# HanielUlises/GCN-GrabCut

Measured on AMD Instinct MI355X. Metric: images/sec end-to-end mask (DUTS-shape batch), higher is better.
Workload: dtype f32

## Files before the change

### gcn-grabcut_amd/csrc/ggc_debug.hip

```cpp
#include "ggc_internal.h"

extern "C" int ggc_debug_read_scratch(ggc_ctx* ctx, const char* name, void* host_dst, size_t bytes) {
    if (!ctx || !name || !host_dst) return GGC_E_INVALID_ARG;
    static const struct { const char* n; int slot; } tab[] = {
        {"slic_raw_labels", ggc::S_SLIC_LABELS}, {"slic_centers", ggc::S_SLIC_CENTERS},
        {"slic_image_a", ggc::S_SLIC_IMG}, {"slic_image_b", ggc::S_SLIC_TMP}, {"slic_stale", ggc::S_SLIC_AUX2},
        {"grabcut_comp", ggc::S_GC_D}, {"grabcut_nweights", ggc::S_GC_E}, {"grabcut_gmm", ggc::S_GC_B},
        {"grabcut_excess_sink_dist", ggc::S_GC_G},
        {"net_states", ggc::S_STATES}, {"net_xw", ggc::S_XW}, {"net_agg", ggc::S_AGG}, {"net_hjk", ggc::S_HJK},
        {"net_score", ggc::S_SCORE}, {"net_gvec", ggc::S_GVEC}, {"net_gate", ggc::S_GATE},
        {"scissors_planes", ggc::S_SCISSORS},
    };
    for (auto& t : tab)
        if (std::strcmp(t.n, name) == 0) {
            const ggc::Buf& b = ctx->slots[t.slot];
            GGC_REQUIRE(ctx, b.p && b.bytes >= bytes, GGC_E_STATE, "scratch '%s' holds %zu bytes, asked for %zu", name,
                        b.bytes, bytes);
            GGC_HIP(ctx, hipSetDevice(ctx->device));
            GGC_HIP(ctx, hipDeviceSynchronize());
            GGC_HIP(ctx, hipMemcpy(host_dst, b.p, bytes, hipMemcpyDeviceToHost));
            return GGC_OK;
        }
    return ggc::set_err(ctx, GGC_E_INVALID_ARG, "unknown scratch name '%s'", name);
}
```

### gcn-grabcut_amd/csrc/ggc_gc.h

```cpp
#pragma once
#include "ggc_internal.h"

namespace ggc {

constexpr int DINF = 1 << 29;

struct GcDims { int B, H, W, P, n_chunks; };

__device__ __forceinline__ int dir_dx(int dir) { return (dir == 0 || dir == 4 || dir == 7) ? -1 : ((dir == 1 || dir == 5 || dir == 6) ? 1 : 0); }
__device__ __forceinline__ int dir_dy(int dir) { return (dir == 2 || dir == 4 || dir == 6) ? -1 : ((dir == 3 || dir == 5 || dir == 7) ? 1 : 0); }
__device__ __forceinline__ int dir_nb(const GcDims& d, int y, int x, int dir) {
    const int yy = y + dir_dy(dir), xx = x + dir_dx(dir);
    if (xx < 0 || xx >= d.W || yy < 0 || yy >= d.H) return -1;
    return yy * d.W + xx;
}

__host__ __device__ __forceinline__ size_t rc_idx(int dir, size_t i) { return i * 8 + (size_t)dir; }

__device__ __forceinline__ void mf_init_pixel(const GcDims& d, int b, int p, int32_t tw, const int32_t* __restrict__ nw,
                                              int32_t* __restrict__ rc, int32_t* __restrict__ ex, int32_t* __restrict__ snk,
                                              uint8_t* __restrict__ rmask, bool warm) {
    const size_t BP = (size_t)d.B * d.P, i = (size_t)b * d.P + p;
    const int y = p / d.W, x = p % d.W;
    const int32_t* nwb = nw + (size_t)b * d.P;
    const int dirs[4] = {0, 4, 2, 6};
    int32_t inflow = 0;
    int arcs = 0;
#pragma unroll
    for (int k = 0; k < 4; ++k) {
        const int dir = dirs[k];
        const int32_t c0 = dir_nb(d, y, x, dir) >= 0 ? nwb[(size_t)k * BP + p] : 0;
        const int q = dir_nb(d, y, x, dir ^ 1);
        const int32_t c1 = q >= 0 ? nwb[(size_t)k * BP + q] : 0;
        if (warm) {
            const int32_t ra = rc[rc_idx(dir, i)], rb = rc[rc_idx((dir ^ 1), i)];
            inflow += (ra - c0) + (rb - c1);
            arcs |= (ra > 0 ? 1 << dir : 0) | (rb > 0 ? 1 << (dir ^ 1) : 0);
        } else {
            rc[rc_idx(dir, i)] = c0;
            rc[rc_idx((dir ^ 1), i)] = c1;
            arcs |= (c0 > 0 ? 1 << dir : 0) | (c1 > 0 ? 1 << (dir ^ 1) : 0);
        }
    }
    rmask[i] = (uint8_t)arcs;
    const int32_t bal = tw + inflow;
    ex[i] = bal > 0 ? bal : 0;
    snk[i] = bal < 0 ? -bal : 0;
}

struct MfControl {
    int32_t* active;
    int32_t* cnt;
    int32_t* lists;
    int32_t* err;
};

int maxflow(ggc_ctx* ctx, hipStream_t st, const GcDims& d, const int32_t* state, int32_t* rc, int32_t* ex,
            int32_t* snk, int32_t* dist, uint8_t* rmask, const MfControl& ctl, bool masks_exact);

constexpr int MF_RT = 32;
constexpr int MF_PT_W = 32, MF_PT_H = 8;
struct MfTiles { int rt_x, rt_y, pt_x, pt_y; };

void mf_zero3(hipStream_t st, int32_t* a, size_t na, int32_t* b, size_t nb, int32_t* c, size_t nc);

constexpr int AQ_HEAD = 0, AQ_TAIL = 32, AQ_PENDING = 64, AQ_DONE = 96, AQ_BUDGET = 97, AQ_VISITS = 128, AQ_WORDS = 160;
int maxflow_relax_async(ggc_ctx* ctx, hipStream_t st, const GcDims& d, const MfTiles& tl, uint8_t* rmask, int32_t* dirty, const int32_t* rc, int32_t* dist,
                        const int32_t* count, const int32_t* list, int32_t* flag, unsigned long long* ring, int32_t* q, int cap,
                        int grid, int32_t* err_flag);
int maxflow_push_async(ggc_ctx* ctx, hipStream_t st, const GcDims& d, const MfTiles& tl, int th, int inner, int gen_max, int32_t* rc,
                       int32_t* ex, int32_t* snk, int32_t* dist, uint8_t* rmask, int32_t* dirty, const int32_t* count, const int32_t* list, int n_list_max, int32_t* state,
                       unsigned long long* ring, int32_t* q, int waves, int32_t* err_flag, long long* prof = nullptr);

}
```

### gcn-grabcut_amd/csrc/ggc_grabcut.hip

```cpp
#include "ggc_gc.h"
#include "ggc_math.h"
#include <algorithm>
#include <cmath>
#include <cstdlib>
#include <vector>

namespace ggc {

constexpr int NCOMP = 5;
constexpr double CAP_SCALE = 262144.0;
constexpr double GAMMA = 50.0, LAMBDA = 9.0 * GAMMA;
constexpr int CHUNK = 1024;


struct Gmm {
    double coef[NCOMP], mean[NCOMP][3], cov[NCOMP][9];
    double inv[NCOMP][3][3], det[NCOMP];
    double isd[NCOMP];
};

__host__ __device__ inline void gmm_prepare(Gmm& g, int ci, double fix) {
    if (!(g.coef[ci] > 0.0)) return;
    double* c = g.cov[ci];
    double d = c[0] * (c[4] * c[8] - c[5] * c[7]) - c[1] * (c[3] * c[8] - c[5] * c[6]) + c[2] * (c[3] * c[7] - c[4] * c[6]);
// ... 182 lines not shown
    }
    const uint64_t r = splitmix(rng);
    const bool by_d2 = k > 0 && total > 0;
    const long long t = by_d2 ? (long long)(r % (uint64_t)total) : (long long)(r % (uint64_t)n);
    const int64_t* w = by_d2 ? cd : cc;
    long long run = 0;
    int ch = d.n_chunks - 1;
    for (int base = 0; base < d.n_chunks; base += 64) {
        const int i = base + lane;
        const long long v = i < d.n_chunks ? (long long)w[i] : 0;
        const long long incl = wave_scan64(v, lane);
        const unsigned long long hit = __ballot(i < d.n_chunks && run + incl > t);
        if (hit) {
            const int l = __ffsll((long long)hit) - 1;
            ch = base + l;
            run += __shfl(incl - v, l, 64);
            break;
        }
        run += __shfl(incl, 63, 64);
    }
    if (ch == d.n_chunks - 1) {
        long long part = 0;
        for (int i = lane; i < d.n_chunks - 1; i += 64) part += w[i];
        run = wave_sum64(part);
    }
    int pick = -1, last = -1;
    const int p_end = min((ch + 1) * CHUNK, d.P);
    for (int base = ch * CHUNK; base < p_end; base += 64) {
        const int p = base + lane;
        const bool mine = p < p_end && (is_bg(mask[(size_t)b * d.P + p]) ? 0 : 1) == c;
        const long long v = mine ? (by_d2 ? (long long)d2[(size_t)b * d.P + p] : 1) : 0;
        const long long incl = wave_scan64(v, lane);
        const unsigned long long any = __ballot(mine);
        if (any) last = base + 63 - __clzll((long long)any);
        const unsigned long long hit = __ballot(mine && run + incl > t);
        if (hit) { pick = base + __ffsll((long long)hit) - 1; break; }
        run += __shfl(incl, 63, 64);
    }
    if (pick < 0) pick = last;
    if (lane == 0) {
        s.rng = rng;
        s.cen_px[k] = pick;
        for (int ch3 = 0; ch3 < 3; ++ch3) s.cen[k][ch3] = (double)img[((size_t)b * d.P + pick) * 3 + ch3];
    }
}

constexpr int ACC_W = 13;

constexpr int BIN_COPIES = 16, BIN_PX = 4;

__global__ void __launch_bounds__(256) k_km_assign(GcDims d, const uint8_t* __restrict__ img,
                                                   const uint8_t* __restrict__ mask, const int32_t* __restrict__ state,
                                                   const KmState* __restrict__ km, uint8_t* __restrict__ comp,
                                                   unsigned long long* __restrict__ acc) {
    __shared__ unsigned int s_acc[2 * NCOMP * 4 * BIN_COPIES];
    const int b = blockIdx.y, tid = threadIdx.x, cp = tid % BIN_COPIES;
    if (state[b]) return;
    for (int i = tid; i < 2 * NCOMP * 4 * BIN_COPIES; i += 256) s_acc[i] = 0;
    __syncthreads();
#pragma unroll
    for (int j = 0; j < BIN_PX; ++j) {
        const int p = (blockIdx.x * BIN_PX + j) * 256 + tid;
        if (p < d.P) {
            const size_t gp = (size_t)b * d.P + p;
            const int c = is_bg(mask[gp]) ? 0 : 1;
            const uint8_t* px = img + gp * 3;
            int best = 0; double bd = 0.0;
#pragma unroll
            for (int cc = 0; cc < 2; ++cc) {
                if (c != cc) continue;
                const KmState& s = km[b * 2 + cc];
                for (int k = 0; k < s.K; ++k) {
                    const double a0 = (double)px[0] - s.cen[k][0], a1 = (double)px[1] - s.cen[k][1], a2 = (double)px[2] - s.cen[k][2];
                    const double dist = (a0 * a0 + a1 * a1) + a2 * a2;
                    if (k == 0 || dist < bd) { best = k; bd = dist; }
                }
            }
            comp[gp] = (uint8_t)best;
            unsigned int* a = s_acc + (c * NCOMP + best) * 4 * BIN_COPIES + cp;
            atomicAdd(&a[0], 1u); atomicAdd(&a[BIN_COPIES], (unsigned int)px[0]);
            atomicAdd(&a[2 * BIN_COPIES], (unsigned int)px[1]); atomicAdd(&a[3 * BIN_COPIES], (unsigned int)px[2]);
        }
    }
    __syncthreads();
    for (int i = tid; i < 2 * NCOMP * 4; i += 256) {
        unsigned int v = 0;
#pragma unroll
        for (int k = 0; k < BIN_COPIES; ++k) v += s_acc[i * BIN_COPIES + k];
        if (v) atomicAdd(&acc[((size_t)b * 2 * NCOMP + i / 4) * ACC_W + (i % 4)], (unsigned long long)v);
    }
}

__global__ void k_km_update(int B, const int32_t* __restrict__ state, KmState* __restrict__ km,
                            unsigned long long* __restrict__ acc, int update) {
    const int i = blockIdx.x * blockDim.x + threadIdx.x;
    if (i >= B * 2 * NCOMP) return;
    const int b = i / (2 * NCOMP), c = (i / NCOMP) % 2, k = i % NCOMP;
    unsigned long long* a = acc + (size_t)i * ACC_W;
    if (!state[b] && update && a[0] > 0)
        for (int ch = 0; ch < 3; ++ch) km[b * 2 + c].cen[k][ch] = (double)(long long)a[1 + ch] / (double)(long long)a[0];
    for (int j = 0; j < ACC_W; ++j) a[j] = 0;
}

template <int MODE>
__global__ void __launch_bounds__(256) k_gmm_accum(GcDims d, const uint8_t* __restrict__ img,
                                                   const uint8_t* __restrict__ mask, const int32_t* __restrict__ state,
                                                   const Gmm* __restrict__ gmm, uint8_t* __restrict__ comp,
                                                   unsigned long long* __restrict__ acc) {
    constexpr int LW = 10;
    __shared__ unsigned int s_acc[2 * NCOMP * LW * BIN_COPIES];
    const int b = blockIdx.y, tid = threadIdx.x, cp = tid % BIN_COPIES;
    if (state[b]) return;
    for (int i = tid; i < 2 * NCOMP * LW * BIN_COPIES; i += 256) s_acc[i] = 0;
    __syncthreads();
#pragma unroll
    for (int j = 0; j < BIN_PX; ++j) {
        const int p = (blockIdx.x * BIN_PX + j) * 256 + tid;
        if (p < d.P) {
            const size_t gp = (size_t)b * d.P + p;
            const int c = is_bg(mask[gp]) ? 0 : 1;
            const uint8_t* px = img + gp * 3;
            int ci = 0;
            if (MODE == 1) {
#pragma unroll
                for (int cc = 0; cc < 2; ++cc) if (c == cc) ci = gmm_which(gmm[b * 2 + cc], px);
                comp[gp] = (uint8_t)ci;
            } else ci = comp[gp];
            unsigned int* a = s_acc + (c * NCOMP + ci) * LW * BIN_COPIES + cp;
            const unsigned int v0 = px[0], v1 = px[1], v2 = px[2];
            atomicAdd(&a[0], 1u);
            atomicAdd(&a[1 * BIN_COPIES], v0); atomicAdd(&a[2 * BIN_COPIES], v1); atomicAdd(&a[3 * BIN_COPIES], v2);
            atomicAdd(&a[4 * BIN_COPIES], v0 * v0); atomicAdd(&a[5 * BIN_COPIES], v0 * v1); atomicAdd(&a[6 * BIN_COPIES], v0 * v2);
            atomicAdd(&a[7 * BIN_COPIES], v1 * v1); atomicAdd(&a[8 * BIN_COPIES], v1 * v2); atomicAdd(&a[9 * BIN_COPIES], v2 * v2);
        }
    }
    __syncthreads();
    for (int i = tid; i < 2 * NCOMP * ACC_W; i += 256) {
        const int bin = i / ACC_W, slot = i % ACC_W;
        int ls = slot;
        if (slot >= 4) {
            const int r = (slot - 4) / 3, cc = (slot - 4) % 3;
            const int lo = r < cc ? r : cc, hi = r < cc ? cc : r;
            ls = 4 + (lo == 0 ? hi : (lo == 1 ? 2 + hi : 5));
        }
        unsigned int v = 0;
#pragma unroll
        for (int k = 0; k < BIN_COPIES; ++k) v += s_acc[(bin * LW + ls) * BIN_COPIES + k];
        if (v) atomicAdd(&acc[(size_t)b * 2 * NCOMP * ACC_W + i], (unsigned long long)v);
    }
}

__global__ void k_gmm_learn(int B, const int32_t* __restrict__ state, unsigned long long* __restrict__ acc,
                            Gmm* __restrict__ gmm) {
    const int i = blockIdx.x * blockDim.x + threadIdx.x;
    if (i >= B * 2) return;
    unsigned long long* a = acc + (size_t)i * NCOMP * ACC_W;
    if (!state[i / 2]) {
        Gmm& g = gmm[i];
        long long total = 0;
        for (int ci = 0; ci < NCOMP; ++ci) total += (long long)a[ci * ACC_W];
        for (int ci = 0; ci < NCOMP; ++ci) {
            const long long n = (long long)a[ci * ACC_W];
            if (n == 0) { g.coef[ci] = 0.0; continue; }
            const double inv_n = 1.0 / (double)n;
            g.coef[ci] = (double)n / (double)total;
            for (int r = 0; r < 3; ++r) g.mean[ci][r] = (double)(long long)a[ci * ACC_W + 1 + r] * inv_n;
            for (int r = 0; r < 3; ++r)
                for (int c = 0; c < 3; ++c)
                    g.cov[ci][3 * r + c] = (double)(long long)a[ci * ACC_W + 4 + 3 * r + c] * inv_n - g.mean[ci][r] * g.mean[ci][c];
            gmm_prepare(g, ci, 0.01);
        }
    }
    for (int j = 0; j < NCOMP * ACC_W; ++j) a[j] = 0;
}

__global__ void k_gmm_from_model(int B, const double* __restrict__ bgd, const double* __restrict__ fgd, Gmm* __restrict__ gmm) {
    const int i = blockIdx.x * blockDim.x + threadIdx.x;
    if (i >= B * 2) return;
    const double* m = (i & 1 ? fgd : bgd) + (size_t)(i / 2) * 65;
    Gmm& g = gmm[i];
    for (int k = 0; k < NCOMP; ++k) g.coef[k] = m[k];
    for (int k = 0; k < 15; ++k) g.mean[k / 3][k % 3] = m[NCOMP + k];
    for (int k = 0; k < 45; ++k) g.cov[k / 9][k % 9] = m[4 * NCOMP + k];
    for (int ci = 0; ci < NCOMP; ++ci) gmm_prepare(g, ci, 0.0);
}

__global__ void k_gmm_to_model(int B, const int32_t* __restrict__ state, const Gmm* __restrict__ gmm,
                               double* __restrict__ bgd, double* __restrict__ fgd) {
    const int i = blockIdx.x * blockDim.x + threadIdx.x;
    if (i >= B * 2 || state[i / 2]) return;
    double* m = (i & 1 ? fgd : bgd) + (size_t)(i / 2) * 65;
    const Gmm& g = gmm[i];
    for (int k = 0; k < NCOMP; ++k) m[k] = g.coef[k];
    for (int k = 0; k < 15; ++k) m[NCOMP + k] = g.mean[k / 3][k % 3];
    for (int k = 0; k < 45; ++k) m[4 * NCOMP + k] = g.cov[k / 9][k % 9];
}

__device__ __forceinline__ bool plane_nb(const GcDims& d, int y, int x, int k, int& q) {
    const int dy = (k == 0) ? 0 : -1, dx = (k == 0 || k == 1) ? -1 : (k == 2 ? 0 : 1);
    const int yy = y + dy, xx = x + dx;
    if (xx < 0 || xx >= d.W || yy < 0) return false;
    q = yy * d.W + xx;
    return true;
}
__device__ __forceinline__ int colour_d2(const uint8_t* a, const uint8_t* b) {
    const int t0 = (int)a[0] - (int)b[0], t1 = (int)a[1] - (int)b[1], t2 = (int)a[2] - (int)b[2];
    return t0 * t0 + t1 * t1 + t2 * t2;
}

__global__ void __launch_bounds__(256) k_beta(GcDims d, const uint8_t* __restrict__ img, unsigned long long* __restrict__ bsum) {
    const int b = blockIdx.y;
    const uint8_t* im = img + (size_t)b * d.P * 3;
    unsigned long long s = 0;
    for (int p = blockIdx.x * blockDim.x + threadIdx.x; p < d.P; p += gridDim.x * blockDim.x) {
        const int y = p / d.W, x = p % d.W;
        for (int k = 0; k < 4; ++k) { int q; if (plane_nb(d, y, x, k, q)) s += (unsigned long long)colour_d2(im + 3 * p, im + 3 * q); }
    }
    for (int o = 32; o > 0; o >>= 1) s += __shfl_xor(s, o, 64);
    if ((threadIdx.x & 63) == 0 && s) atomicAdd(&bsum[b], s);
}

__global__ void __launch_bounds__(256) k_nweights(GcDims d, const uint8_t* __restrict__ img,
                                                  const unsigned long long* __restrict__ bsum, int32_t* __restrict__ nw) {
    const size_t i = (size_t)blockIdx.x * blockDim.x + threadIdx.x;
    if (i >= (size_t)d.B * d.P) return;
    const int b = (int)(i / d.P), p = (int)(i % d.P);
    const int y = p / d.W, x = p % d.W;
    const uint8_t* im = img + (size_t)b * d.P * 3;
    const long long bs = (long long)bsum[b];
    double beta = 0.0;
    if (bs > 0) beta = 1.0 / (2.0 * (double)bs / (double)(4ll * d.W * d.H - 3ll * d.W - 3ll * d.H + 2));
    const double gdiv = GAMMA / sqrt(2.0);
    for (int k = 0; k < 4; ++k) {
        int q; int32_t w = 0;
        if (plane_nb(d, y, x, k, q)) {
            const double wt = ((k & 1) ? gdiv : GAMMA) * det_exp(-beta * (double)colour_d2(im + 3 * p, im + 3 * q));
            w = (int32_t)rint(wt * CAP_SCALE);
        }
        nw[((size_t)k * d.B + b) * d.P + p] = w;
    }
}

__global__ void __launch_bounds__(256) k_build_graph(GcDims d, const uint8_t* __restrict__ img,
                                                     const uint8_t* __restrict__ mask, const int32_t* __restrict__ state,
                                                     const Gmm* __restrict__ gmm, const int32_t* __restrict__ nw,
                                                     int32_t* __restrict__ rc, int32_t* __restrict__ ex,
                                                     int32_t* __restrict__ snk, uint8_t* __restrict__ rmask, int warm) {
    const int b = blockIdx.y, p = blockIdx.x * blockDim.x + threadIdx.x;
    if (p >= d.P || state[b]) return;
    const size_t i = (size_t)b * d.P + p;
    const uint8_t m = mask[i];
    if (warm && (m == GGC_BGD || m == GGC_FGD)) return;
    double dv;
    if (m == GGC_BGD) dv = -LAMBDA;
    else if (m == GGC_FGD) dv = LAMBDA;
    else {
        const uint8_t* px = img + i * 3;
        const double from_src = -det_log(gmm_total(gmm[b * 2 + 0], px));
        const double to_snk = -det_log(gmm_total(gmm[b * 2 + 1], px));
        dv = from_src - to_snk;
        if (dv != dv) dv = 0.0;
        if (dv > LAMBDA) dv = LAMBDA;
        if (dv < -LAMBDA) dv = -LAMBDA;
    }
    mf_init_pixel(d, b, p, (int32_t)rint(dv * CAP_SCALE), nw, rc, ex, snk, rmask, warm != 0);
}

__global__ void __launch_bounds__(256) k_gc_relabel(GcDims d, const int32_t* __restrict__ state,
                                                    const int32_t* __restrict__ dist, uint8_t* __restrict__ mask) {
    const size_t i = (size_t)blockIdx.x * blockDim.x + threadIdx.x;
    if (i >= (size_t)d.B * d.P || state[i / d.P]) return;
    const uint8_t m = mask[i];
    if (m == GGC_PR_BGD || m == GGC_PR_FGD) mask[i] = dist[i] >= DINF ? GGC_PR_FGD : GGC_PR_BGD;
}

__global__ void __launch_bounds__(256) k_gc_binary(size_t n, const uint8_t* __restrict__ mask, uint8_t* __restrict__ binary) {
    const size_t i = (size_t)blockIdx.x * blockDim.x + threadIdx.x;
    if (i < n) binary[i] = (mask[i] == GGC_FGD || mask[i] == GGC_PR_FGD) ? 1 : 0;
}

}

using namespace ggc;

extern "C" int ggc_grabcut(ggc_ctx* ctx, ggc_stream stream, int B, int H, int W, const uint8_t* image,
                           uint8_t* mask, const int32_t* rects, double* bgd_model, double* fgd_model,
                           int n_iter, int mode, uint64_t seed, uint8_t* binary) {
    if (!ctx) return GGC_E_INVALID_ARG;
    GGC_REQUIRE(ctx, B >= 1 && H >= 1 && W >= 1 && B <= 65535, GGC_E_SHAPE, "bad shape B=%d H=%d W=%d", B, H, W);
    GGC_REQUIRE(ctx, (size_t)H * W < (1u << 28), GGC_E_SHAPE, "image too large");
    GGC_REQUIRE(ctx, image && mask, GGC_E_INVALID_ARG, "null pointer");
    GGC_REQUIRE(ctx, mode >= 0 && mode <= 2, GGC_E_INVALID_ARG, "mode must be 0 (mask), 1 (rect) or 2 (eval)");
    GGC_REQUIRE(ctx, mode != 1 || rects, GGC_E_INVALID_ARG, "mode 1 needs rects");
    GGC_REQUIRE(ctx, mode != 2 || (bgd_model && fgd_model), GGC_E_INVALID_ARG, "mode 2 needs both models");
    GGC_HIP(ctx, hipSetDevice(ctx->device));
    hipStream_t st = reinterpret_cast<hipStream_t>(stream);
    GcDims d{B, H, W, H * W, cdiv((size_t)H * W, CHUNK)};
    const size_t BP = (size_t)B * d.P;

    int32_t *f1, *f2, *state, *err;
    MfControl mf;
    const size_t ctl_bytes = carve_scratch(ctx, S_GC_A, [&](Carve& c) {
        f1 = c.take<int32_t>(B); f2 = c.take<int32_t>(B); state = c.take<int32_t>(B); err = c.take<int32_t>(2);
        mf = {c.take<int32_t>(B), c.take<int32_t>(8), c.take<int32_t>(2 * (size_t)B), err ? err + 1 : nullptr};
    });
    Gmm* gmm = scratch_t<Gmm>(ctx, S_GC_B, (size_t)B * 2);
    unsigned long long* acc = scratch_t<unsigned long long>(ctx, S_GC_C, (size_t)B * 2 * NCOMP * ACC_W + B);
    uint8_t* comp = scratch_t<uint8_t>(ctx, S_GC_D, BP);
    int32_t* nw = scratch_t<int32_t>(ctx, S_GC_E, BP * 4);
    int32_t* rc = scratch_t<int32_t>(ctx, S_GC_F, BP * 8);
    int32_t* ex = scratch_t<int32_t>(ctx, S_GC_G, BP * 3);
    uint8_t* rmask = scratch_t<uint8_t>(ctx, S_GC_L, BP);
    if (!ctl_bytes || !gmm || !acc || !comp || !nw || !rc || !ex || !rmask) return GGC_E_OOM;
    int32_t* snk = ex + BP;
    int32_t* dist = ex + 2 * BP;
    unsigned long long* bsum = acc + (size_t)B * 2 * NCOMP * ACC_W;
    GGC_HIP(ctx, hipMemsetAsync(f1, 0, ctl_bytes, st));
    GGC_HIP(ctx, hipMemsetAsync(acc, 0, sizeof(unsigned long long) * ((size_t)B * 2 * NCOMP * ACC_W + B), st));

    if (mode == 1) {
        int32_t* drects = scratch_t<int32_t>(ctx, S_GC_H, (size_t)B * 4);
        if (!drects) return GGC_E_OOM;
        GGC_HIP(ctx, hipMemcpyAsync(drects, rects, sizeof(int32_t) * B * 4, hipMemcpyHostToDevice, st));
        hipLaunchKernelGGL(k_gc_rect, dim3(cdiv(BP, 256)), dim3(256), 0, st, d, drects, mask);
    }
    const dim3 red(std::min(cdiv(d.P, 256 * 4), 128), B);
    hipLaunchKernelGGL(k_gc_flags, red, dim3(256), 0, st, d, mask, f1);
    if (mode == 0) hipLaunchKernelGGL(k_gc_promote, dim3(cdiv(BP, 256)), dim3(256), 0, st, d, f1, mask);
    hipLaunchKernelGGL(k_gc_flags, red, dim3(256), 0, st, d, mask, f2);
    hipLaunchKernelGGL(k_gc_state, dim3(cdiv(B, 256)), dim3(256), 0, st, B, mode, f1, f2, state, err);
    GGC_LAUNCH_CHECK(ctx);

    if (mode == 2) {
        hipLaunchKernelGGL(k_gmm_from_model, dim3(cdiv(B * 2, 64)), dim3(64), 0, st, B, bgd_model, fgd_model, gmm);
    } else {
        ProfScope prof(ctx, st, "grabcut_init_gmm");
        KmState* km = scratch_t<KmState>(ctx, S_GC_I, (size_t)B * 2);
        int32_t* d2 = scratch_t<int32_t>(ctx, S_GC_J, BP);
        int64_t* chunks = scratch_t<int64_t>(ctx, S_GC_K, (size_t)B * 2 * d.n_chunks * 2);
        if (!km || !d2 || !chunks) return GGC_E_OOM;
        int64_t* chunk_cnt = chunks;
        int64_t* chunk_d2 = chunks + (size_t)B * 2 * d.n_chunks;
        for (int k = 0; k < NCOMP; ++k) {
            hipLaunchKernelGGL(k_km_chunks, dim3(d.n_chunks, B), dim3(256), 0, st, d, k, image, mask, state, km, d2, chunk_cnt, chunk_d2);
            hipLaunchKernelGGL(k_km_pick, dim3(B), dim3(128), 0, st, d, k, (uint64_t)seed, image, mask, state, d2, chunk_cnt, chunk_d2, km);
        }
        for (int it = 0; it < 10; ++it) {
            hipLaunchKernelGGL(k_km_assign, dim3(cdiv(d.P, 256 * BIN_PX), B), dim3(256), 0, st, d, image, mask, state, km, comp, acc);
            hipLaunchKernelGGL(k_km_update, dim3(cdiv(B * 2 * NCOMP, 256)), dim3(256), 0, st, B, state, km, acc, it < 9 ? 1 : 0);
        }
        hipLaunchKernelGGL((k_gmm_accum<0>), dim3(cdiv(d.P, 256 * BIN_PX), B), dim3(256), 0, st, d, image, mask, state, gmm, comp, acc);
        hipLaunchKernelGGL(k_gmm_learn, dim3(cdiv(B * 2, 64)), dim3(64), 0, st, B, state, acc, gmm);
    }
    GGC_LAUNCH_CHECK(ctx);

    if (n_iter > 0) {
        hipLaunchKernelGGL(k_beta, red, dim3(256), 0, st, d, image, bsum);
        hipLaunchKernelGGL(k_nweights, dim3(cdiv(BP, 256)), dim3(256), 0, st, d, image, bsum, nw);
        GGC_LAUNCH_CHECK(ctx);
        for (int it = 0; it < n_iter; ++it) {
            const bool warm = knobs().mf_warm && it > 0;
            {
                ProfScope prof(ctx, st, "grabcut_gmm");
                hipLaunchKernelGGL((k_gmm_accum<1>), dim3(cdiv(d.P, 256 * BIN_PX), B), dim3(256), 0, st, d, image, mask, state, gmm, comp, acc);
                hipLaunchKernelGGL(k_gmm_learn, dim3(cdiv(B * 2, 64)), dim3(64), 0, st, B, state, acc, gmm);
                hipLaunchKernelGGL(k_build_graph, dim3(cdiv(d.P, 256), B), dim3(256), 0, st, d, image, mask, state, gmm, nw, rc, ex, snk, rmask, warm ? 1 : 0);
            }
            GGC_LAUNCH_CHECK(ctx);
            const int rcode = maxflow(ctx, st, d, state, rc, ex, snk, dist, rmask, mf, !warm);
            if (rcode) return rcode;
            hipLaunchKernelGGL(k_gc_relabel, dim3(cdiv(BP, 256)), dim3(256), 0, st, d, state, dist, mask);
            GGC_LAUNCH_CHECK(ctx);
        }
    }
    if (bgd_model && fgd_model)
        hipLaunchKernelGGL(k_gmm_to_model, dim3(cdiv(B * 2, 64)), dim3(64), 0, st, B, state, gmm, bgd_model, fgd_model);
    if (binary) hipLaunchKernelGGL(k_gc_binary, dim3(cdiv(BP, 256)), dim3(256), 0, st, BP, mask, binary);
    GGC_LAUNCH_CHECK(ctx);
    std::vector<int32_t> herr;
    int rcode = read_i32(ctx, st, err, 2, herr);
    if (rcode) return rcode;
    GGC_REQUIRE(ctx, herr[0] == 0, GGC_E_INVALID_ARG, "mask holds values outside {0,1,2,3}");
    GGC_REQUIRE(ctx, herr[1] == 0, GGC_E_DEVICE, "max-flow did not converge (code %d)", herr[1]);
    return GGC_OK;
}
```

### gcn-grabcut_amd/csrc/ggc_gridflow.hip

```cpp
#include "ggc_gc.h"
#include <algorithm>
#include <vector>

namespace ggc {
namespace {

constexpr int32_t GF_TW_MAX = 1 << 27;
constexpr int32_t GF_NW_MAX = 1 << 24;

__global__ void __launch_bounds__(256) k_gf_check(GcDims d, int n_steps, const int32_t* __restrict__ tw,
                                                  const int32_t* __restrict__ nw, int32_t* __restrict__ err) {
    const size_t BP = (size_t)d.B * d.P, i = (size_t)blockIdx.x * 256 + threadIdx.x;
    int bad = 0;
    if (i < BP) {
        const int p = (int)(i % d.P), y = p / d.W, x = p % d.W;
        for (int s = 0; s < n_steps; ++s) {
            const int32_t t = tw[(size_t)s * BP + i];
            bad |= (t < -GF_TW_MAX || t > GF_TW_MAX) ? 1 : 0;
        }
        const int dirs[4] = {0, 4, 2, 6};
#pragma unroll
        for (int k = 0; k < 4; ++k) {
            if (dir_nb(d, y, x, dirs[k]) < 0) continue;
            const int32_t w = nw[(size_t)k * BP + i];
            bad |= (w < 0 ? 2 : 0) | (w > GF_NW_MAX ? 4 : 0);
        }
    }
    for (int o = 32; o > 0; o >>= 1) bad |= __shfl_xor(bad, o, 64);
    if ((threadIdx.x & 63) == 0 && bad) atomicOr(err, bad);
}

__global__ void __launch_bounds__(256) k_gf_build(GcDims d, const int32_t* __restrict__ tw, const int32_t* __restrict__ nw,
                                                  int32_t* __restrict__ rc, int32_t* __restrict__ ex, int32_t* __restrict__ snk,
                                                  uint8_t* __restrict__ rmask, int warm) {
    const int b = blockIdx.y, p = blockIdx.x * blockDim.x + threadIdx.x;
    if (p >= d.P) return;
    mf_init_pixel(d, b, p, tw[(size_t)b * d.P + p], nw, rc, ex, snk, rmask, warm != 0);
}

__global__ void __launch_bounds__(256) k_gf_side(size_t n, const int32_t* __restrict__ dist, uint8_t* __restrict__ side) {
    const size_t i = (size_t)blockIdx.x * 256 + threadIdx.x;
    if (i < n) side[i] = dist[i] >= DINF ? 1 : 0;
}

__global__ void __launch_bounds__(256) k_gf_residual(size_t n, const int32_t* __restrict__ rc, const int32_t* __restrict__ ex,
                                                     const int32_t* __restrict__ snk, int32_t* __restrict__ out) {
    const size_t i = (size_t)blockIdx.x * 256 + threadIdx.x;
    if (i >= n) return;
#pragma unroll
    for (int dir = 0; dir < 8; ++dir) out[i * 10 + dir] = rc[rc_idx(dir, i)];
    out[i * 10 + 8] = ex[i];
    out[i * 10 + 9] = snk[i];
}

}
}

using namespace ggc;

extern "C" int ggc_grid_maxflow(ggc_ctx* ctx, ggc_stream stream, int B, int H, int W, int n_steps, const int32_t* tw,
                                const int32_t* nw, uint8_t* source_side, int32_t* residual) {
    if (!ctx) return GGC_E_INVALID_ARG;
    GGC_REQUIRE(ctx, B >= 1 && H >= 1 && W >= 1 && B <= 65535, GGC_E_INVALID_ARG, "bad shape B=%d H=%d W=%d", B, H, W);
    GGC_REQUIRE(ctx, (size_t)H * W < (1u << 28), GGC_E_SHAPE, "image too large");
    GGC_REQUIRE(ctx, n_steps >= 1, GGC_E_INVALID_ARG, "n_steps must be >= 1 (got %d)", n_steps);
    GGC_REQUIRE(ctx, tw && nw && source_side, GGC_E_INVALID_ARG, "null pointer");
    GGC_HIP(ctx, hipSetDevice(ctx->device));
    hipStream_t st = reinterpret_cast<hipStream_t>(stream);
    GcDims d{B, H, W, H * W, 0};
    const size_t BP = (size_t)B * d.P;

    int32_t *state, *err;
    MfControl mf;
    const size_t ctl_bytes = carve_scratch(ctx, S_GC_A, [&](Carve& c) {
        state = c.take<int32_t>(B); err = c.take<int32_t>(2);
        mf = {c.take<int32_t>(B), c.take<int32_t>(8), c.take<int32_t>(2 * (size_t)B), err ? err + 1 : nullptr};
    });
    int32_t* rc = scratch_t<int32_t>(ctx, S_GC_F, BP * 8);
    int32_t* ex = scratch_t<int32_t>(ctx, S_GC_G, BP * 3);
    uint8_t* rmask = scratch_t<uint8_t>(ctx, S_GC_L, BP);
    if (!ctl_bytes || !rc || !ex || !rmask) return GGC_E_OOM;
    int32_t* snk = ex + BP;
    int32_t* dist = ex + 2 * BP;
    GGC_HIP(ctx, hipMemsetAsync(state, 0, ctl_bytes, st));

    hipLaunchKernelGGL(k_gf_check, dim3(cdiv(BP, 256)), dim3(256), 0, st, d, n_steps, tw, nw, err);
    GGC_LAUNCH_CHECK(ctx);
    std::vector<int32_t> herr;
    int rcode = read_i32(ctx, st, err, 1, herr);
    if (rcode) return rcode;
    GGC_REQUIRE(ctx, !(herr[0] & 1), GGC_E_INVALID_ARG, "a t-link difference lies outside [-2^27, 2^27]");
    GGC_REQUIRE(ctx, !(herr[0] & 2), GGC_E_INVALID_ARG, "an in-image n-link is negative");
    GGC_REQUIRE(ctx, !(herr[0] & 4), GGC_E_INVALID_ARG, "an in-image n-link exceeds 2^24");

    for (int s = 0; s < n_steps; ++s) {
        const bool warm = knobs().mf_warm && s > 0;
        hipLaunchKernelGGL(k_gf_build, dim3(cdiv(d.P, 256), B), dim3(256), 0, st, d, tw + (size_t)s * BP, nw, rc, ex, snk, rmask, warm ? 1 : 0);
        GGC_LAUNCH_CHECK(ctx);
        if ((rcode = maxflow(ctx, st, d, state, rc, ex, snk, dist, rmask, mf, !warm))) return rcode;
        hipLaunchKernelGGL(k_gf_side, dim3(cdiv(BP, 256)), dim3(256), 0, st, BP, dist, source_side + (size_t)s * BP);
        GGC_LAUNCH_CHECK(ctx);
        if ((rcode = read_i32(ctx, st, err + 1, 1, herr))) return rcode;
        GGC_REQUIRE(ctx, herr[0] == 0, GGC_E_DEVICE, "max-flow did not converge in step %d (code %d)", s, herr[0]);
    }
    if (residual) {
        hipLaunchKernelGGL(k_gf_residual, dim3(cdiv(BP, 256)), dim3(256), 0, st, BP, rc, ex, snk, residual);
        GGC_LAUNCH_CHECK(ctx);
    }
    GGC_HIP(ctx, hipStreamSynchronize(st));
    return GGC_OK;
}
```

### gcn-grabcut_amd/csrc/ggc_maxflow.hip

```cpp
#include "ggc_gc.h"
#include "ggc_mf_sweep.h"
#include <algorithm>
#include <chrono>
#include <cstdlib>
#include <vector>

namespace ggc {

constexpr int RT = MF_RT;
constexpr int PT_W = MF_PT_W, PT_H = MF_PT_H;
constexpr int PT_N = PT_W * PT_H;
constexpr int PUSH_GRID = 1024, RELAX_GRID = 1024, ASYNC_GRID = 128;

__global__ void __launch_bounds__(256) k_mf_zero3(int32_t* __restrict__ a, size_t na, int32_t* __restrict__ b, size_t nb, int32_t* __restrict__ c, size_t nc) {
    const size_t i = (size_t)blockIdx.x * 256 + threadIdx.x;
    if (i < na) a[i] = 0;
    else if (i < na + nb) b[i - na] = 0;
    else if (i < na + nb + nc) c[i - na - nb] = 0;
}
void mf_zero3(hipStream_t st, int32_t* a, size_t na, int32_t* b, size_t nb, int32_t* c, size_t nc) {
    const size_t n = na + nb + nc;
    if (n) hipLaunchKernelGGL(k_mf_zero3, dim3(cdiv(n, 256)), dim3(256), 0, st, a, na, b, nb, c, nc);
}

// ... 401 lines not shown
struct MfTrace {
    std::chrono::steady_clock::time_point t_prev = std::chrono::steady_clock::now();
    double push_ms = 0.0;

    int round(const MfSolve& s, int round, int n_next, int total_active, int relax_launches) {
        ggc_ctx* ctx = s.ctx;
        long long hh[64 * 8], h[7] = {0, 0, 0, 0, 0, 0, 0};
        GGC_HIP(ctx, hipStreamSynchronize(s.st));
        GGC_HIP(ctx, hipMemcpy(hh, s.prof + 64 * 8, sizeof hh, hipMemcpyDeviceToHost));
        GGC_HIP(ctx, hipMemsetAsync(s.prof + 64 * 8, 0, sizeof hh, s.st));
        for (int i = 0; i < 64; ++i) for (int k = 0; k < 7; ++k) h[k] += hh[i * 8 + k];
        if (h[3] > 0)
            std::fprintf(stderr, "    [relabel visits] %lld dense visits: per visit load+fill %.2f us, sweeps %.2f us (%.1f sweeps, %.1f BFS levels, %lld visits fell back), write-back %.2f us\n",
                         h[3], 0.01 * h[0] / h[3], 0.01 * h[1] / h[3], (double)h[4] / h[3], (double)h[5] / h[3], h[6], 0.01 * h[2] / h[3]);
        std::vector<int32_t> act;
        if (int rcode = read_i32(ctx, s.st, s.ctl.active, s.d.B, act)) return rcode;
        const auto t_now = std::chrono::steady_clock::now();
        const double ms = std::chrono::duration<double, std::milli>(t_now - t_prev).count();
        std::fprintf(stderr, "[ggc maxflow] round %d: open images %d, active pixels %d, relabel launches %d, relabel+scan %.3f ms, previous push %.3f ms\n",
                     round, n_next, total_active, relax_launches, ms - push_ms, push_ms);
        t_prev = t_now;
        if (n_next > 0 && n_next <= 12) {
            std::fprintf(stderr, "    [open]");
            for (int b = 0; b < s.d.B; ++b) if (act[b]) std::fprintf(stderr, " %d:%d", b, act[b]);
            std::fprintf(stderr, "\n");
        }
        return GGC_OK;
    }

    int push(const MfSolve& s, int waves) {
        ggc_ctx* ctx = s.ctx;
        GGC_HIP(ctx, hipStreamSynchronize(s.st));
        push_ms = std::chrono::duration<double, std::milli>(std::chrono::steady_clock::now() - t_prev).count();
        if (waves == 0) return GGC_OK;
        long long hh[128 * 8], h[7] = {0, 0, 0, 0, 0, 0, 0}, g[3] = {0, 0, 0};
        GGC_HIP(ctx, hipMemcpy(hh, s.prof, sizeof hh, hipMemcpyDeviceToHost));
        GGC_HIP(ctx, hipMemsetAsync(s.prof, 0, sizeof hh, s.st));
        for (int i = 0; i < 64; ++i) for (int k = 0; k < 7; ++k) h[k] += hh[i * 8 + k];
        for (int i = 0; i < 64; ++i) for (int k = 0; k < 3; ++k) g[k] += hh[(64 + i) * 8 + k];
        if (h[3] > 0)
            std::fprintf(stderr, "    [async visit] load+fill %.2f us, sweeps %.2f us (%.1f sweeps), write-back+drain %.2f us\n", 0.01 * g[0] / h[3],
                         0.01 * g[1] / h[3], (double)g[2] / h[3], 0.01 * (h[1] - g[0] - g[1]) / h[3]);
        if (h[6] > 0)
            std::fprintf(stderr, "    [async push] %d waves alive %.1f us on average; %lld visits (%lld followed): per visit wait+lock %.2f us, "
                         "visit %.2f us, hand-over %.2f us\n", waves, 0.01 * h[5] / h[6], h[3], h[4], h[3] ? 0.01 * h[0] / h[3] : 0.0,
                         h[3] ? 0.01 * h[1] / h[3] : 0.0, h[3] ? 0.01 * h[2] / h[3] : 0.0);
        return GGC_OK;
    }
};

}

int maxflow(ggc_ctx* ctx, hipStream_t st, const GcDims& d, const int32_t* state, int32_t* rc, int32_t* ex,
            int32_t* snk, int32_t* dist, uint8_t* rmask, const MfControl& ctl, bool masks_exact) {
    const Knobs& kn = knobs();
    const MfTiles tl{cdiv(d.W, RT), cdiv(d.H, RT), cdiv(d.W, PT_W), cdiv(d.H, PT_H)};
    MfSolve s{ctx, st, d, tl, (size_t)tl.rt_x * tl.rt_y * d.B, (size_t)tl.pt_x * tl.pt_y * d.B, rc, ex, snk, dist, rmask,
              ctl, ctl.cnt, ctl.cnt + 1, ctl.cnt + 4, {}, nullptr};
    GGC_REQUIRE(ctx, std::max(s.n_rt, s.n_pt) < (1u << 24), GGC_E_UNSUPPORTED, "batch has more max-flow tiles than a queue entry addresses");
    if (!carve_scratch(ctx, S_GC_M, [&](Carve& c) { s.w.layout(c, s.n_rt, s.n_pt); })) return GGC_E_OOM;
    if (masks_exact) GGC_HIP(ctx, hipMemsetAsync(s.w.dirty, 0, sizeof(int32_t) * s.n_pt, st));
    if (kn.mf_trace) {
        s.prof = s.w.prof;
        GGC_HIP(ctx, hipMemsetAsync(s.prof, 0, 2 * 64 * 8 * sizeof(long long), st));
    }
    GGC_HIP(ctx, hipMemsetAsync(s.n_open, 0, sizeof(int32_t), st));
    int32_t *list_cur = ctl.lists, *list_nxt = ctl.lists + d.B;
    hipLaunchKernelGGL(k_open_init, dim3(cdiv(d.B, 256)), dim3(256), 0, st, d.B, state, list_cur, s.n_open, s.rl_cnt);
    GGC_LAUNCH_CHECK(ctx);
    std::vector<int32_t> host;
    int rcode = read_i32(ctx, st, s.n_open, 1, host);
    if (rcode) return rcode;
    int n_cur = host[0];
    if (n_cur == 0) return GGC_OK;
    MfTrace trace;
    const int max_rounds = 4096;
    for (int round = 0; round < max_rounds; ++round) {
        const size_t scale = std::max<size_t>(1, ((size_t)n_cur + 32) / 64);
        const bool partial = round < kn.mf_partial_rounds;
        int relax_launches = 0;
        if ((rcode = s.relabel(list_cur, n_cur, scale, partial, relax_launches))) return rcode;
        hipLaunchKernelGGL(k_mf_active, dim3(std::min(cdiv(tl.pt_x * tl.pt_y, 4), 128), n_cur), dim3(256), 0, st, d, tl, list_cur, ex, dist,
                           ctl.active, s.w.pt_flag[0], s.w.pt_flag[1], s.w.pt_list[0], s.pr_cnt);
        hipLaunchKernelGGL(k_done_update, dim3(cdiv(n_cur, 256)), dim3(256), 0, st, n_cur, list_cur, ctl.active, list_nxt, s.n_open, partial ? 1 : 0, s.rl_cnt);
        GGC_LAUNCH_CHECK(ctx);
        if ((rcode = read_i32(ctx, st, s.n_open, 8, host))) return rcode;
        const int n_next = host[0], total_active = host[7];
        if (kn.mf_trace && (rcode = trace.round(s, round, n_next, total_active, relax_launches))) return rcode;
        if (n_next == 0) return GGC_OK;
        std::swap(list_cur, list_nxt);
        int waves = 0;
        if ((rcode = s.push(round, n_cur, scale, total_active, waves))) return rcode;
        if (kn.mf_trace && (rcode = trace.push(s, waves))) return rcode;
        n_cur = n_next;
    }
    return set_err(ctx, GGC_E_DEVICE, "max-flow did not converge in %d rounds", max_rounds);
}

}
```

Measured before the change: 3777.

## Fuse n-link weights into graph build, warm-start t-link deltas, trim redundant passes

Drops the separate n-weights kernel and its 4-plane buffer. Cold graph builds now compute 8-neighbour capacities inline and write them as int4 stores, and warm builds update excess and sink from the change in t-link weight instead of re-reading residual capacities. The per-iteration relabel kernel and the comp store in the GMM pass are folded into the next GMM accumulation, which relabels the mask from dist. K-means stores comp only on its last iteration. The host readback of the open-image count is cached across max-flow calls, which saves a sync but assumes the number of open images stays the same between iterations.

```diff
diff --git a/gcn-grabcut_amd/csrc/ggc_debug.hip b/gcn-grabcut_amd/csrc/ggc_debug.hip
--- a/gcn-grabcut_amd/csrc/ggc_debug.hip
+++ b/gcn-grabcut_amd/csrc/ggc_debug.hip
@@ -5,7 +5,7 @@
     static const struct { const char* n; int slot; } tab[] = {
         {"slic_raw_labels", ggc::S_SLIC_LABELS}, {"slic_centers", ggc::S_SLIC_CENTERS},
         {"slic_image_a", ggc::S_SLIC_IMG}, {"slic_image_b", ggc::S_SLIC_TMP}, {"slic_stale", ggc::S_SLIC_AUX2},
-        {"grabcut_comp", ggc::S_GC_D}, {"grabcut_nweights", ggc::S_GC_E}, {"grabcut_gmm", ggc::S_GC_B},
+        {"grabcut_comp", ggc::S_GC_D}, {"grabcut_tlinks", ggc::S_GC_E}, {"grabcut_gmm", ggc::S_GC_B},
         {"grabcut_excess_sink_dist", ggc::S_GC_G},
         {"net_states", ggc::S_STATES}, {"net_xw", ggc::S_XW}, {"net_agg", ggc::S_AGG}, {"net_hjk", ggc::S_HJK},
         {"net_score", ggc::S_SCORE}, {"net_gvec", ggc::S_GVEC}, {"net_gate", ggc::S_GATE},
diff --git a/gcn-grabcut_amd/csrc/ggc_gc.h b/gcn-grabcut_amd/csrc/ggc_gc.h
--- a/gcn-grabcut_amd/csrc/ggc_gc.h
+++ b/gcn-grabcut_amd/csrc/ggc_gc.h
@@ -17,33 +17,36 @@
 
 __host__ __device__ __forceinline__ size_t rc_idx(int dir, size_t i) { return i * 8 + (size_t)dir; }
 
-__device__ __forceinline__ void mf_init_pixel(const GcDims& d, int b, int p, int32_t tw, const int32_t* __restrict__ nw,
-                                              int32_t* __restrict__ rc, int32_t* __restrict__ ex, int32_t* __restrict__ snk,
-                                              uint8_t* __restrict__ rmask, bool warm) {
-    const size_t BP = (size_t)d.B * d.P, i = (size_t)b * d.P + p;
+__device__ __forceinline__ void mf_cold_pixel(size_t i, int32_t tw, const int32_t (&cap)[8], int32_t* __restrict__ rc,
+                                              int32_t* __restrict__ ex, int32_t* __restrict__ snk, uint8_t* __restrict__ rmask) {
+    int arcs = 0;
+    int4* r = reinterpret_cast<int4*>(rc + rc_idx(0, i));
+    r[0] = make_int4(cap[0], cap[1], cap[2], cap[3]);
+    r[1] = make_int4(cap[4], cap[5], cap[6], cap[7]);
+#pragma unroll
+    for (int dir = 0; dir < 8; ++dir) arcs |= cap[dir] > 0 ? 1 << dir : 0;
+    rmask[i] = (uint8_t)arcs;
+    ex[i] = tw > 0 ? tw : 0;
+    snk[i] = tw < 0 ? -tw : 0;
+}
+
+__device__ __forceinline__ void mf_plane_caps(const GcDims& d, int b, int p, const int32_t* __restrict__ nw, int32_t (&cap)[8]) {
+    const size_t BP = (size_t)d.B * d.P;
     const int y = p / d.W, x = p % d.W;
     const int32_t* nwb = nw + (size_t)b * d.P;
     const int dirs[4] = {0, 4, 2, 6};
-    int32_t inflow = 0;
-    int arcs = 0;
 #pragma unroll
     for (int k = 0; k < 4; ++k) {
         const int dir = dirs[k];
-        const int32_t c0 = dir_nb(d, y, x, dir) >= 0 ? nwb[(size_t)k * BP + p] : 0;
+        cap[dir] = dir_nb(d, y, x, dir) >= 0 ? nwb[(size_t)k * BP + p] : 0;
         const int q = dir_nb(d, y, x, dir ^ 1);
-        const int32_t c1 = q >= 0 ? nwb[(size_t)k * BP + q] : 0;
-        if (warm) {
-            const int32_t ra = rc[rc_idx(dir, i)], rb = rc[rc_idx((dir ^ 1), i)];
-            inflow += (ra - c0) + (rb - c1);
-            arcs |= (ra > 0 ? 1 << dir : 0) | (rb > 0 ? 1 << (dir ^ 1) : 0);
-        } else {
-            rc[rc_idx(dir, i)] = c0;
-            rc[rc_idx((dir ^ 1), i)] = c1;
-            arcs |= (c0 > 0 ? 1 << dir : 0) | (c1 > 0 ? 1 << (dir ^ 1) : 0);
-        }
+        cap[dir ^ 1] = q >= 0 ? nwb[(size_t)k * BP + q] : 0;
     }
-    rmask[i] = (uint8_t)arcs;
-    const int32_t bal = tw + inflow;
+}
+
+__device__ __forceinline__ void mf_warm_pixel(size_t i, int32_t tw, int32_t tw_old, int32_t* __restrict__ ex,
+                                              int32_t* __restrict__ snk) {
+    const int32_t bal = (ex[i] - snk[i]) + (tw - tw_old);
     ex[i] = bal > 0 ? bal : 0;
     snk[i] = bal < 0 ? -bal : 0;
 }
@@ -56,7 +59,7 @@
 };
 
 int maxflow(ggc_ctx* ctx, hipStream_t st, const GcDims& d, const int32_t* state, int32_t* rc, int32_t* ex,
-            int32_t* snk, int32_t* dist, uint8_t* rmask, const MfControl& ctl, bool masks_exact);
+            int32_t* snk, int32_t* dist, uint8_t* rmask, const MfControl& ctl, bool masks_exact, int& n_open);
 
 constexpr int MF_RT = 32;
 constexpr int MF_PT_W = 32, MF_PT_H = 8;
diff --git a/gcn-grabcut_amd/csrc/ggc_grabcut.hip b/gcn-grabcut_amd/csrc/ggc_grabcut.hip
--- a/gcn-grabcut_amd/csrc/ggc_grabcut.hip
+++ b/gcn-grabcut_amd/csrc/ggc_grabcut.hip
@@ -258,7 +258,7 @@
 __global__ void __launch_bounds__(256) k_km_assign(GcDims d, const uint8_t* __restrict__ img,
                                                    const uint8_t* __restrict__ mask, const int32_t* __restrict__ state,
                                                    const KmState* __restrict__ km, uint8_t* __restrict__ comp,
-                                                   unsigned long long* __restrict__ acc) {
+                                                   unsigned long long* __restrict__ acc, int store_comp) {
     __shared__ unsigned int s_acc[2 * NCOMP * 4 * BIN_COPIES];
     const int b = blockIdx.y, tid = threadIdx.x, cp = tid % BIN_COPIES;
     if (state[b]) return;
@@ -282,7 +282,7 @@
                     if (k == 0 || dist < bd) { best = k; bd = dist; }
                 }
             }
-            comp[gp] = (uint8_t)best;
+            if (store_comp) comp[gp] = (uint8_t)best;
             unsigned int* a = s_acc + (c * NCOMP + best) * 4 * BIN_COPIES + cp;
             atomicAdd(&a[0], 1u); atomicAdd(&a[BIN_COPIES], (unsigned int)px[0]);
             atomicAdd(&a[2 * BIN_COPIES], (unsigned int)px[1]); atomicAdd(&a[3 * BIN_COPIES], (unsigned int)px[2]);
@@ -310,9 +310,9 @@
 
 template <int MODE>
 __global__ void __launch_bounds__(256) k_gmm_accum(GcDims d, const uint8_t* __restrict__ img,
-                                                   const uint8_t* __restrict__ mask, const int32_t* __restrict__ state,
-                                                   const Gmm* __restrict__ gmm, uint8_t* __restrict__ comp,
-                                                   unsigned long long* __restrict__ acc) {
+                                                   uint8_t* __restrict__ mask, const int32_t* __restrict__ state,
+                                                   const Gmm* __restrict__ gmm, const uint8_t* __restrict__ comp,
+                                                   const int32_t* __restrict__ dist, unsigned long long* __restrict__ acc) {
     constexpr int LW = 10;
     __shared__ unsigned int s_acc[2 * NCOMP * LW * BIN_COPIES];
     const int b = blockIdx.y, tid = threadIdx.x, cp = tid % BIN_COPIES;
@@ -324,13 +324,17 @@
         const int p = (blockIdx.x * BIN_PX + j) * 256 + tid;
         if (p < d.P) {
             const size_t gp = (size_t)b * d.P + p;
-            const int c = is_bg(mask[gp]) ? 0 : 1;
+            uint8_t m = mask[gp];
+            if (MODE == 1 && dist && (m == GGC_PR_BGD || m == GGC_PR_FGD)) {
+                const uint8_t m1 = dist[gp] >= DINF ? GGC_PR_FGD : GGC_PR_BGD;
+                if (m1 != m) mask[gp] = m = m1;
+            }
+            const int c = is_bg(m) ? 0 : 1;
             const uint8_t* px = img + gp * 3;
             int ci = 0;
             if (MODE == 1) {
 #pragma unroll
                 for (int cc = 0; cc < 2; ++cc) if (c == cc) ci = gmm_which(gmm[b * 2 + cc], px);
-                comp[gp] = (uint8_t)ci;
             } else ci = comp[gp];
             unsigned int* a = s_acc + (c * NCOMP + ci) * LW * BIN_COPIES + cp;
             const unsigned int v0 = px[0], v1 = px[1], v2 = px[2];
@@ -426,32 +430,22 @@
     if ((threadIdx.x & 63) == 0 && s) atomicAdd(&bsum[b], s);
 }
 
-__global__ void __launch_bounds__(256) k_nweights(GcDims d, const uint8_t* __restrict__ img,
-                                                  const unsigned long long* __restrict__ bsum, int32_t* __restrict__ nw) {
-    const size_t i = (size_t)blockIdx.x * blockDim.x + threadIdx.x;
-    if (i >= (size_t)d.B * d.P) return;
-    const int b = (int)(i / d.P), p = (int)(i % d.P);
-    const int y = p / d.W, x = p % d.W;
-    const uint8_t* im = img + (size_t)b * d.P * 3;
-    const long long bs = (long long)bsum[b];
-    double beta = 0.0;
-    if (bs > 0) beta = 1.0 / (2.0 * (double)bs / (double)(4ll * d.W * d.H - 3ll * d.W - 3ll * d.H + 2));
+__device__ __forceinline__ double gc_beta(const GcDims& d, unsigned long long bsum) {
+    const long long bs = (long long)bsum;
+    return bs > 0 ? 1.0 / (2.0 * (double)bs / (double)(4ll * d.W * d.H - 3ll * d.W - 3ll * d.H + 2)) : 0.0;
+}
+__device__ __forceinline__ int32_t nlink_cap(double beta, bool diagonal, const uint8_t* a, const uint8_t* b) {
     const double gdiv = GAMMA / sqrt(2.0);
-    for (int k = 0; k < 4; ++k) {
-        int q; int32_t w = 0;
-        if (plane_nb(d, y, x, k, q)) {
-            const double wt = ((k & 1) ? gdiv : GAMMA) * det_exp(-beta * (double)colour_d2(im + 3 * p, im + 3 * q));
-            w = (int32_t)rint(wt * CAP_SCALE);
-        }
-        nw[((size_t)k * d.B + b) * d.P + p] = w;
-    }
+    const double wt = (diagonal ? gdiv : GAMMA) * det_exp(-beta * (double)colour_d2(a, b));
+    return (int32_t)rint(wt * CAP_SCALE);
 }
 
 __global__ void __launch_bounds__(256) k_build_graph(GcDims d, const uint8_t* __restrict__ img,
                                                      const uint8_t* __restrict__ mask, const int32_t* __restrict__ state,
-                                                     const Gmm* __restrict__ gmm, const int32_t* __restrict__ nw,
+                                                     const Gmm* __restrict__ gmm, const unsigned long long* __restrict__ bsum,
                                                      int32_t* __restrict__ rc, int32_t* __restrict__ ex,
-                                                     int32_t* __restrict__ snk, uint8_t* __restrict__ rmask, int warm) {
+                                                     int32_t* __restrict__ snk, uint8_t* __restrict__ rmask,
+                                                     int32_t* __restrict__ tws, int warm) {
     const int b = blockIdx.y, p = blockIdx.x * blockDim.x + threadIdx.x;
     if (p >= d.P || state[b]) return;
     const size_t i = (size_t)b * d.P + p;
@@ -469,7 +463,21 @@
         if (dv > LAMBDA) dv = LAMBDA;
         if (dv < -LAMBDA) dv = -LAMBDA;
     }
-    mf_init_pixel(d, b, p, (int32_t)rint(dv * CAP_SCALE), nw, rc, ex, snk, rmask, warm != 0);
+    const int32_t tw = (int32_t)rint(dv * CAP_SCALE);
+    if (warm) mf_warm_pixel(i, tw, tws[i], ex, snk);
+    else {
+        const uint8_t* im = img + (size_t)b * d.P * 3;
+        const double beta = gc_beta(d, bsum[b]);
+        const int y = p / d.W, x = p % d.W;
+        int32_t cap[8];
+#pragma unroll
+        for (int dir = 0; dir < 8; ++dir) {
+            const int q = dir_nb(d, y, x, dir);
+            cap[dir] = q >= 0 ? nlink_cap(beta, dir >= 4, im + 3 * p, im + 3 * q) : 0;
+        }
+        mf_cold_pixel(i, tw, cap, rc, ex, snk, rmask);
+    }
+    tws[i] = tw;
 }
 
 __global__ void __launch_bounds__(256) k_gc_relabel(GcDims d, const int32_t* __restrict__ state,
@@ -513,11 +521,11 @@
     Gmm* gmm = scratch_t<Gmm>(ctx, S_GC_B, (size_t)B * 2);
     unsigned long long* acc = scratch_t<unsigned long long>(ctx, S_GC_C, (size_t)B * 2 * NCOMP * ACC_W + B);
     uint8_t* comp = scratch_t<uint8_t>(ctx, S_GC_D, BP);
-    int32_t* nw = scratch_t<int32_t>(ctx, S_GC_E, BP * 4);
+    int32_t* tws = scratch_t<int32_t>(ctx, S_GC_E, BP);
     int32_t* rc = scratch_t<int32_t>(ctx, S_GC_F, BP * 8);
     int32_t* ex = scratch_t<int32_t>(ctx, S_GC_G, BP * 3);
     uint8_t* rmask = scratch_t<uint8_t>(ctx, S_GC_L, BP);
-    if (!ctl_bytes || !gmm || !acc || !comp || !nw || !rc || !ex || !rmask) return GGC_E_OOM;
+    if (!ctl_bytes || !gmm || !acc || !comp || !tws || !rc || !ex || !rmask) return GGC_E_OOM;
     int32_t* snk = ex + BP;
     int32_t* dist = ex + 2 * BP;
     unsigned long long* bsum = acc + (size_t)B * 2 * NCOMP * ACC_W;
@@ -552,30 +560,31 @@
             hipLaunchKernelGGL(k_km_pick, dim3(B), dim3(128), 0, st, d, k, (uint64_t)seed, image, mask, state, d2, chunk_cnt, chunk_d2, km);
         }
         for (int it = 0; it < 10; ++it) {
-            hipLaunchKernelGGL(k_km_assign, dim3(cdiv(d.P, 256 * BIN_PX), B), dim3(256), 0, st, d, image, mask, state, km, comp, acc);
+            hipLaunchKernelGGL(k_km_assign, dim3(cdiv(d.P, 256 * BIN_PX), B), dim3(256), 0, st, d, image, mask, state, km, comp, acc, it == 9 ? 1 : 0);
             hipLaunchKernelGGL(k_km_update, dim3(cdiv(B * 2 * NCOMP, 256)), dim3(256), 0, st, B, state, km, acc, it < 9 ? 1 : 0);
         }
-        hipLaunchKernelGGL((k_gmm_accum<0>), dim3(cdiv(d.P, 256 * BIN_PX), B), dim3(256), 0, st, d, image, mask, state, gmm, comp, acc);
+        hipLaunchKernelGGL((k_gmm_accum<0>), dim3(cdiv(d.P, 256 * BIN_PX), B), dim3(256), 0, st, d, image, mask, state, gmm, comp, (const int32_t*)nullptr, acc);
         hipLaunchKernelGGL(k_gmm_learn, dim3(cdiv(B * 2, 64)), dim3(64), 0, st, B, state, acc, gmm);
     }
     GGC_LAUNCH_CHECK(ctx);
 
     if (n_iter > 0) {
         hipLaunchKernelGGL(k_beta, red, dim3(256), 0, st, d, image, bsum);
-        hipLaunchKernelGGL(k_nweights, dim3(cdiv(BP, 256)), dim3(256), 0, st, d, image, bsum, nw);
         GGC_LAUNCH_CHECK(ctx);
+        int n_open = -1;
         for (int it = 0; it < n_iter; ++it) {
             const bool warm = knobs().mf_warm && it > 0;
             {
                 ProfScope prof(ctx, st, "grabcut_gmm");
-                hipLaunchKernelGGL((k_gmm_accum<1>), dim3(cdiv(d.P, 256 * BIN_PX), B), dim3(256), 0, st, d, image, mask, state, gmm, comp, acc);
+                hipLaunchKernelGGL((k_gmm_accum<1>), dim3(cdiv(d.P, 256 * BIN_PX), B), dim3(256), 0, st, d, image, mask, state, gmm, comp,
+                                   (const int32_t*)(it > 0 ? dist : nullptr), acc);
                 hipLaunchKernelGGL(k_gmm_learn, dim3(cdiv(B * 2, 64)), dim3(64), 0, st, B, state, acc, gmm);
-                hipLaunchKernelGGL(k_build_graph, dim3(cdiv(d.P, 256), B), dim3(256), 0, st, d, image, mask, state, gmm, nw, rc, ex, snk, rmask, warm ? 1 : 0);
+                hipLaunchKernelGGL(k_build_graph, dim3(cdiv(d.P, 256), B), dim3(256), 0, st, d, image, mask, state, gmm, bsum, rc, ex, snk, rmask, tws, warm ? 1 : 0);
             }
             GGC_LAUNCH_CHECK(ctx);
-            const int rcode = maxflow(ctx, st, d, state, rc, ex, snk, dist, rmask, mf, !warm);
+            const int rcode = maxflow(ctx, st, d, state, rc, ex, snk, dist, rmask, mf, !warm, n_open);
             if (rcode) return rcode;
-            hipLaunchKernelGGL(k_gc_relabel, dim3(cdiv(BP, 256)), dim3(256), 0, st, d, state, dist, mask);
+            if (it == n_iter - 1) hipLaunchKernelGGL(k_gc_relabel, dim3(cdiv(BP, 256)), dim3(256), 0, st, d, state, dist, mask);
             GGC_LAUNCH_CHECK(ctx);
         }
     }
diff --git a/gcn-grabcut_amd/csrc/ggc_gridflow.hip b/gcn-grabcut_amd/csrc/ggc_gridflow.hip
--- a/gcn-grabcut_amd/csrc/ggc_gridflow.hip
+++ b/gcn-grabcut_amd/csrc/ggc_gridflow.hip
@@ -30,12 +30,16 @@
     if ((threadIdx.x & 63) == 0 && bad) atomicOr(err, bad);
 }
 
-__global__ void __launch_bounds__(256) k_gf_build(GcDims d, const int32_t* __restrict__ tw, const int32_t* __restrict__ nw,
-                                                  int32_t* __restrict__ rc, int32_t* __restrict__ ex, int32_t* __restrict__ snk,
-                                                  uint8_t* __restrict__ rmask, int warm) {
+__global__ void __launch_bounds__(256) k_gf_build(GcDims d, const int32_t* __restrict__ tw, const int32_t* __restrict__ tw_old,
+                                                  const int32_t* __restrict__ nw, int32_t* __restrict__ rc, int32_t* __restrict__ ex,
+                                                  int32_t* __restrict__ snk, uint8_t* __restrict__ rmask) {
     const int b = blockIdx.y, p = blockIdx.x * blockDim.x + threadIdx.x;
     if (p >= d.P) return;
-    mf_init_pixel(d, b, p, tw[(size_t)b * d.P + p], nw, rc, ex, snk, rmask, warm != 0);
+    const size_t i = (size_t)b * d.P + p;
+    if (tw_old) { mf_warm_pixel(i, tw[i], tw_old[i], ex, snk); return; }
+    int32_t cap[8];
+    mf_plane_caps(d, b, p, nw, cap);
+    mf_cold_pixel(i, tw[i], cap, rc, ex, snk, rmask);
 }
 
 __global__ void __launch_bounds__(256) k_gf_side(size_t n, const int32_t* __restrict__ dist, uint8_t* __restrict__ side) {
@@ -93,11 +97,13 @@
     GGC_REQUIRE(ctx, !(herr[0] & 2), GGC_E_INVALID_ARG, "an in-image n-link is negative");
     GGC_REQUIRE(ctx, !(herr[0] & 4), GGC_E_INVALID_ARG, "an in-image n-link exceeds 2^24");
 
+    int n_open = -1;
     for (int s = 0; s < n_steps; ++s) {
         const bool warm = knobs().mf_warm && s > 0;
-        hipLaunchKernelGGL(k_gf_build, dim3(cdiv(d.P, 256), B), dim3(256), 0, st, d, tw + (size_t)s * BP, nw, rc, ex, snk, rmask, warm ? 1 : 0);
+        const int32_t* tw_s = tw + (size_t)s * BP;
+        hipLaunchKernelGGL(k_gf_build, dim3(cdiv(d.P, 256), B), dim3(256), 0, st, d, tw_s, warm ? tw_s - BP : nullptr, nw, rc, ex, snk, rmask);
         GGC_LAUNCH_CHECK(ctx);
-        if ((rcode = maxflow(ctx, st, d, state, rc, ex, snk, dist, rmask, mf, !warm))) return rcode;
+        if ((rcode = maxflow(ctx, st, d, state, rc, ex, snk, dist, rmask, mf, !warm, n_open))) return rcode;
         hipLaunchKernelGGL(k_gf_side, dim3(cdiv(BP, 256)), dim3(256), 0, st, BP, dist, source_side + (size_t)s * BP);
         GGC_LAUNCH_CHECK(ctx);
         if ((rcode = read_i32(ctx, st, err + 1, 1, herr))) return rcode;
diff --git a/gcn-grabcut_amd/csrc/ggc_maxflow.hip b/gcn-grabcut_amd/csrc/ggc_maxflow.hip
--- a/gcn-grabcut_amd/csrc/ggc_maxflow.hip
+++ b/gcn-grabcut_amd/csrc/ggc_maxflow.hip
@@ -477,7 +477,7 @@
 }
 
 int maxflow(ggc_ctx* ctx, hipStream_t st, const GcDims& d, const int32_t* state, int32_t* rc, int32_t* ex,
-            int32_t* snk, int32_t* dist, uint8_t* rmask, const MfControl& ctl, bool masks_exact) {
+            int32_t* snk, int32_t* dist, uint8_t* rmask, const MfControl& ctl, bool masks_exact, int& n_open) {
     const Knobs& kn = knobs();
     const MfTiles tl{cdiv(d.W, RT), cdiv(d.H, RT), cdiv(d.W, PT_W), cdiv(d.H, PT_H)};
     MfSolve s{ctx, st, d, tl, (size_t)tl.rt_x * tl.rt_y * d.B, (size_t)tl.pt_x * tl.pt_y * d.B, rc, ex, snk, dist, rmask,
@@ -494,9 +494,12 @@
     hipLaunchKernelGGL(k_open_init, dim3(cdiv(d.B, 256)), dim3(256), 0, st, d.B, state, list_cur, s.n_open, s.rl_cnt);
     GGC_LAUNCH_CHECK(ctx);
     std::vector<int32_t> host;
-    int rcode = read_i32(ctx, st, s.n_open, 1, host);
-    if (rcode) return rcode;
-    int n_cur = host[0];
+    int rcode = GGC_OK;
+    if (n_open < 0) {
+        if ((rcode = read_i32(ctx, st, s.n_open, 1, host))) return rcode;
+        n_open = host[0];
+    }
+    int n_cur = n_open;
     if (n_cur == 0) return GGC_OK;
     MfTrace trace;
     const int max_rounds = 4096;
```

Measured after the change: 3816, median of 6. 1.0% higher.
